# bitsandbytes-foundation/bitsandbytes

Measured on AMD Instinct MI355X. Metric: NF4 gemv_4bit / Linear4bit decode forward GB/s (M=1, N=K=4096; algorithmic bytes / time), higher is better.
Workload: dtype bf16

## Files before the change

### bitsandbytes_amd/cextension.py

```python
from __future__ import annotations

import ctypes as ct
import logging
import os
from pathlib import Path

logger = logging.getLogger(__name__)

PACKAGE_DIR = Path(__file__).resolve().parent
LIB_NAME = "libbitsandbytes_mi355x.so"
LIB_PATH = Path(os.environ.get("BNB_MI355X_LIBRARY", PACKAGE_DIR / LIB_NAME))


class MissingNativeLibrary:

    def __init__(self, reason: str):
        self._reason = reason

    def __getattr__(self, name):
        raise RuntimeError(
            f"bitsandbytes_amd: native symbol '{name}' requested but {LIB_NAME} is not loaded ({self._reason}). "
            f"Build it with `make -C {PACKAGE_DIR / 'csrc'}` (needs hipcc, targets gfx950). "
            "There is no CPU or PyTorch fallback for the 4-bit kernels in this package."
        )
# ... 42 lines not shown
    sig(["bnb_mi355x_gemm_4bit_grad_input_workspace_bytes"], [_I32] * 3, ct.c_size_t)
    sig(["bnb_mi355x_gemm_4bit_grad_input_supported"], [_I32] * 5, _I32)
    sig(["bnb_mi355x_peer_buffer_bytes"], [_I32, ct.c_size_t], ct.c_size_t)
    sig(["bnb_mi355x_peer_alloc"], [ct.c_size_t], _VOID_P)
    sig(["bnb_mi355x_peer_free", "bnb_mi355x_peer_close"], [_VOID_P])
    sig(["bnb_mi355x_peer_export"], [_VOID_P, _VOID_P], _I32)
    sig(["bnb_mi355x_peer_open"], [_VOID_P], _VOID_P)
    sig(["bnb_mi355x_peer_allgather"], [_VOID_P, _I32, _I32, _VOID_P, _VOID_P, ct.c_size_t, ct.c_size_t, _VOID_P])
    sig(["bnb_mi355x_peer_status"], [_VOID_P], _I32)
    sig(["bnb_mi355x_peer_chain_buffer_bytes"], [ct.c_long], ct.c_size_t)
    sig(["bnb_mi355x_peer_chain_alloc"], [ct.c_size_t, _I32], _VOID_P)
    sig(["bnb_mi355x_gemv_4bit_peer_serves"], [_I32] * 5 + [ct.c_long, _I32], _I32)
    sig(["bnb_mi355x_gemv_4bit_peer"], [_VOID_P, _VOID_P, _I32, _I32, _I32] + [_VOID_P] * 8 + [_I32] * 5 + [ct.c_long, _I32, _I32, _VOID_P], _I32)
    sig(["bnb_mi355x_peer_chain_read"], [_VOID_P, _VOID_P, _I32, _I32, _I32, _VOID_P, _I32, ct.c_long, _I32, _VOID_P])
    sig(["bnb_mi355x_set_stream_tuning"], [_I32] * 5)
    sig(["bnb_mi355x_set_tuning"], [_I32] * 4)
    sig(["bnb_mi355x_set_stamp_buffer"], [_VOID_P])
    sig(["bnb_mi355x_version"], [], ct.c_char_p)


def load_native_library():
    if not LIB_PATH.exists():
        return MissingNativeLibrary(f"{LIB_PATH} does not exist")
    try:
        dll = ct.CDLL(str(LIB_PATH))
        _declare(dll)
    except (OSError, AttributeError) as exc:
        logger.error("bitsandbytes_amd: failed to load %s: %s", LIB_PATH, exc)
        return MissingNativeLibrary(str(exc))
    return dll
# ... 5 lines not shown
    [f"cquantize_blockwise_{d}_{q}" for d in ("fp32", "bf16", "fp16") for q in ("nf4", "fp4")]
    + [f"cdequantize_blockwise_{d}_{q}" for d in ("fp32", "bf16", "fp16") for q in ("nf4", "fp4")]
    + [f"cquantize_blockwise_{d}" for d in ("fp32", "bf16", "fp16")]
    + [f"cdequantize_blockwise_{d}" for d in ("fp32", "bf16", "fp16")]
    + [f"cgemm_4bit_{d}" for d in ("fp32", "bf16", "fp16")]
    + [f"cgemm_4bit_inference_naive_{d}" for d in ("fp32", "bf16", "fp16")]
    + ["get_context", "cget_managed_ptr", "bnb_mi355x_quantize_4bit", "bnb_mi355x_quantize_8bit", "bnb_mi355x_quantize_4bit_nested", "bnb_mi355x_dequantize_4bit_nested", "bnb_mi355x_dequantize_4bit_rows",
       "bnb_mi355x_gemm_4bit", "bnb_mi355x_gemm_4bit_workspace_bytes", "bnb_mi355x_gemm_4bit_route", "bnb_mi355x_last_gemm_kernel",
       "bnb_mi355x_gemm_4bit_grouped", "bnb_mi355x_gemm_4bit_grouped_route",
       "bnb_mi355x_gemm_4bit_experts", "bnb_mi355x_gemm_4bit_experts_supported",
       "bnb_mi355x_gemm_4bit_grad_input", "bnb_mi355x_gemm_4bit_grad_input_workspace_bytes", "bnb_mi355x_gemm_4bit_grad_input_supported",
       "bnb_mi355x_peer_buffer_bytes", "bnb_mi355x_peer_alloc", "bnb_mi355x_peer_free", "bnb_mi355x_peer_export", "bnb_mi355x_peer_open",
       "bnb_mi355x_peer_close", "bnb_mi355x_peer_allgather", "bnb_mi355x_peer_status",
       "bnb_mi355x_peer_chain_buffer_bytes", "bnb_mi355x_peer_chain_alloc", "bnb_mi355x_gemv_4bit_peer_serves", "bnb_mi355x_gemv_4bit_peer",
       "bnb_mi355x_peer_chain_read",
       "bnb_mi355x_set_stream_tuning", "bnb_mi355x_set_tuning", "bnb_mi355x_set_stamp_buffer", "bnb_mi355x_version"]
)
```

### bitsandbytes_amd/csrc/c_api.hip

```cpp
#include "bnb_common.h"

#include "../../include/bnb_mi355x.h"

namespace bnb {
void quantize_4bit_f32(const float*, float*, uint8_t*, int, long, int, hipStream_t);
void quantize_4bit_f16(const void*, float*, uint8_t*, int, long, int, hipStream_t);
void quantize_4bit_bf16(const void*, float*, uint8_t*, int, long, int, hipStream_t);
void dequantize_4bit_f32(const uint8_t*, const float*, float*, int, long, int, hipStream_t);
void dequantize_4bit_rows(int, const uint8_t*, const float*, const void*, int, void*, long, long, int, int, int, hipStream_t);
void dequantize_4bit_f16(const uint8_t*, const float*, void*, int, long, int, hipStream_t);
void dequantize_4bit_bf16(const uint8_t*, const float*, void*, int, long, int, hipStream_t);
void quantize_8bit_f32(const float*, const float*, float*, uint8_t*, int, long, hipStream_t);
void quantize_8bit_f16(const float*, const void*, float*, uint8_t*, int, long, hipStream_t);
void quantize_8bit_bf16(const float*, const void*, float*, uint8_t*, int, long, hipStream_t);
void dequantize_8bit_f32(const float*, const uint8_t*, const float*, float*, int, long, hipStream_t);
void dequantize_8bit_f16(const float*, const uint8_t*, const float*, void*, int, long, hipStream_t);
void dequantize_8bit_bf16(const float*, const uint8_t*, const float*, void*, int, long, hipStream_t);
void gemv_4bit_stream(int dtype, const void* A, const uint8_t* B, const float* absmax, const uint8_t* absmax8,
                      const float* absmax_code, const float* absmax_offset, const float* code16, void* out,
                      const void* bias, int M, int N, int K, int blocksize, int quant_type, hipStream_t stream);
bool gemv_4bit_grouped(int dtype, const void* A, int count, const uint8_t* const* B, const float* const* absmax,
                       const uint8_t* const* absmax8, const float* const* absmax_code, const float* const* absmax_offset,
                       void* const* out, const void* const* bias, const int* N, int M, int K, int blocksize, int quant_type,
                       hipStream_t stream);
void gemv_4bit_stream_tuning(int ns, int sw, int rows_per_wg, int nt, int waves);
bool gemv_4bit_peer(void* const* bufs, void* epoch_word, int world, int rank, int dtype, const void* A, const uint8_t* B, const float* absmax,
                    const uint8_t* absmax8, const float* absmax_code, const float* absmax_offset, const void* bias, void* out_local,
                    int ns, int K, int blocksize, int quant_type, int mode, long max_values, int wg_limit, uint32_t epoch_offset,
                    uint32_t spin_bound, hipStream_t stream);
void peer_chain_read(void* const* bufs, void* epoch_word, int world, int rank, int dtype, void* out, int nvalues, long max_values, uint32_t epoch_offset,
                     uint32_t spin_bound, hipStream_t stream);
bool gemv_4bit_peer_serves(int world, int ns, int K, int blocksize, int mode, long max_values, int wg_limit);
thread_local int g_last_gemm_kernel = kKernelNone;
#ifdef BNB_PROFILING
unsigned long long* g_dbg_buf = nullptr;
#endif
bool gemm_4bit_mfma_supported(int dtype, const void* A, const uint8_t* B, const float* code16, int M, int N, int K, int blocksize, bool plain_absmax);
void gemm_4bit_mfma(int dtype, const void* A, const uint8_t* B, const float* absmax, const uint8_t* absmax8,
                    const float* absmax_code, const float* absmax_offset, const float* code16, void* out,
                    const void* bias, int M, int N, int K, int blocksize, int quant_type, void* workspace,
// ... 375 lines not shown
int bnb_mi355x_gemm_4bit_grad_input_supported(int dtype, int M, int N, int K, int blocksize) {
    static const int dummy_aligned[4] __attribute__((aligned(16))) = {0, 0, 0, 0};
    return gemm_4bit_grad_input_supported(dtype, dummy_aligned, reinterpret_cast<const uint8_t*>(dummy_aligned), M, N, K, blocksize) ? 1 : 0;
}
void bnb_mi355x_set_tuning(int reserved0, int reserved1, int mfma_knob0, int mfma_knob1) {
    quantize_8bit_set_variant(reserved0);
    quantize_4bit_set_variant(reserved0 == 3 ? 1 : reserved0 == 4 ? 4 : reserved0 == 5 ? 3 : reserved0 == 8 ? 2 : 0);
    dequantize_4bit_set_variant(reserved0 >= 10 ? reserved0 - 10 : 0);
    gemm_4bit_grad_input_set_slices(reserved1);
    g_mfma_knob0.store(mfma_knob0, std::memory_order_relaxed);
    g_mfma_knob1.store(mfma_knob1, std::memory_order_relaxed);
}
void bnb_mi355x_set_stream_tuning(int ring_depth, int segments, int rows_per_workgroup, int nontemporal, int waves) {
    gemv_4bit_stream_tuning(ring_depth, segments, rows_per_workgroup, nontemporal, waves);
}
void bnb_mi355x_set_stamp_buffer(void* device_u64_buffer) {
#ifdef BNB_PROFILING
    g_dbg_buf = static_cast<unsigned long long*>(device_u64_buffer);
#else
    (void)device_u64_buffer;
#endif
}
const char* bnb_mi355x_version(void) { return "bitsandbytes_amd 0.1.1 gfx950"; }

#pragma GCC visibility pop
}
```

### bitsandbytes_amd/csrc/gemm4_mfma_sm.hip

```cpp
#include "bnb_common.h"

namespace bnb {

#ifdef BNB_PROFILING
extern unsigned long long* g_dbg_buf;
#endif

namespace {

using u32x4 = __attribute__((ext_vector_type(4))) uint32_t;
using f32x4 = __attribute__((ext_vector_type(4))) float;
using i32x4 = __attribute__((ext_vector_type(4))) int;

template <typename T> struct SmMma;
template <> struct SmMma<bf16> {
    using frag = __attribute__((ext_vector_type(8))) bf16;
    static __device__ __forceinline__ f32x4 run(u32x4 a, u32x4 b, f32x4 c) {
        return __builtin_amdgcn_mfma_f32_16x16x32_bf16(__builtin_bit_cast(frag, a), __builtin_bit_cast(frag, b), c, 0, 0, 0);
    }
    static __device__ __forceinline__ uint32_t pack(float first, float second) {
        using V = __attribute__((ext_vector_type(2))) bf16;
        V v;
        v[0] = static_cast<bf16>(first);
        v[1] = static_cast<bf16>(second);
// ... 238 lines not shown
        asm volatile("" : "+s"(ob));
        offset = __builtin_bit_cast(float, ob);
    }

    const int mrow = ln & (SROWS - 1);
    const uint32_t frag_base = stage_lds + static_cast<uint32_t>(mrow * 512) +
                               static_cast<uint32_t>(((4 * (lg & 1) + 2 * (lg >> 1)) ^ sm_swz(mrow)) << 4);
    u32x4 af[8];
    auto read_frags = [&]() {
#pragma unroll
        for (int s = 0; s < 8; ++s) {
            const uint32_t sbits = static_cast<uint32_t>(256 * (s >> 2) + 128 * ((s >> 1) & 1) + 16 * (s & 1));
            af[s] = *reinterpret_cast<const __attribute__((address_space(3))) u32x4*>(frag_base ^ sbits);
        }
    };
    __syncthreads();
    BNB_SM_STAMP(5)
    if constexpr (!SINGLE) {
        issue(st[1], 1);
        __builtin_amdgcn_sched_barrier(0);
    }
    if constexpr (ORDER == 1)
        sm_wait_vm<0>();
    else
        sm_wait_vm<NS * LPS>();
    BNB_SM_STAMP(3)
    read_frags();
    if constexpr (!SINGLE) {
        if (nchunks > 1) {
            sm_wait_lgkm0();
// ... 340 lines not shown
```

### bitsandbytes_amd/csrc/gemv4_stream.hip

```cpp
#include "bnb_common.h"

#include <type_traits>

namespace bnb {

#ifdef BNB_PROFILING
extern unsigned long long* g_dbg_buf;
#endif

namespace {

using u32x4 = __attribute__((ext_vector_type(4))) uint32_t;
using f32x2 = __attribute__((ext_vector_type(2))) float;
using f32x4 = __attribute__((ext_vector_type(4))) float;

typedef __attribute__((address_space(3))) unsigned char* lds_ptr;

constexpr int kSegK = 2048;
constexpr int kLutBytes = 65536;
constexpr int kMaxGroup = 8;

enum StreamFlags : int {
    kNested = 1,
    kCodePtr = 2,
    kFp4 = 4,
    kNT = 8,
    kGrouped = 16,
    kMulti = 32,
    kPeer = 64
};

struct StreamMat {
    const uint8_t* B;
    const float* absmax;
    const uint8_t* absmax8;
    const float* absmax_code;
    const float* absmax_offset;
    void* out;
    const void* bias;
    int N;
    int row_start;
};

#ifdef BNB_PROFILING
// ... 68 lines not shown
    for (int i = 0; i < 4; ++i) {
        const uint32_t e = v[i];
        dst[i] = __builtin_bit_cast(float, e);
    }
}

template <typename T, int MB, int WAVES, int NS, int FLAGS>
__global__ __launch_bounds__(WAVES * 64) __attribute__((amdgpu_waves_per_eu(WAVES / 4, WAVES / 4))) void gemv4_stream_kernel(
    const void* hot_A, const uint8_t* hot_B, const float* hot_absmax, const uint8_t* hot_absmax8, int hot_N, int hot_K,
    int hot_packed , int hot_geom ,
    int hot_inv , const StreamArgs p) {
    constexpr bool NESTED = FLAGS & kNested, CODEPTR = FLAGS & kCodePtr, NT = FLAGS & kNT, GROUPED = FLAGS & kGrouped;
    constexpr bool MULTI = FLAGS & kMulti;
    constexpr bool PEER = (FLAGS & kPeer) != 0;
    static_assert(!PEER || (MB == 1 && !MULTI && !GROUPED && WAVES == 16), "the peer-chain form is the M = 1, single-phase kernel");
    constexpr int THREADS = WAVES * 64;
    constexpr int TB = TypeInfo<T>::bytes;
    constexpr int CH = 2 * TB;
    constexpr int EPC = 16 / TB;
    constexpr int LPS = 2;
    constexpr int BUILDERS = (WAVES >= 16) ? WAVES / 2 : WAVES;
    constexpr int IL = (NS % 2 == 0 && WAVES < 16 && MB <= 2) ? 2 : 1;
    static_assert(NS % IL == 0, "the ring is consumed IL stages at a time");

    extern __shared__ __attribute__((aligned(16))) unsigned char smem[];
    const int tid = threadIdx.x;
    const int lane = tid & 63;
    const int wave = __builtin_amdgcn_readfirstlane(tid >> 6);
    const int K = hot_K;
    const int M = hot_packed & 0x3FFFF, bs_shift = (hot_packed >> 18) & 31, P = MULTI ? (hot_packed >> 23) & 511 : 1;
    const int R = hot_geom & 0xFFFF, SW = (hot_geom >> 16) & 31, G = (hot_geom >> 21) & 31;
    const int S = (K + kSegK - 1) >> 11;
    const int rows_total = GROUPED ? p.rows_total : hot_N;
    const int row_begin = blockIdx.x * R;
    if (row_begin >= rows_total)
        return;
    const int nrows = (rows_total - row_begin < R) ? rows_total - row_begin : R;
    const int m0 = blockIdx.y * MB;
    const int g = (wave * hot_inv) >> 8;
    const int sw = wave - g * SW;
#ifdef BNB_PROFILING
    if (p.dbg && lane == 0)
        BNB_ST_DBG_BASE[(static_cast<long>(blockIdx.x) * WAVES + wave) * 16 + 13] = __builtin_amdgcn_s_memrealtime();
#endif
    BNB_ST_STAMP(0)

    constexpr int kCode2Bytes = (GROUPED ? kMaxGroup : 1) * 1024 + 64;
    float* const code2 = reinterpret_cast<float*>(smem + kLutBytes);
    unsigned char* const ximg = smem + kLutBytes + kCode2Bytes;
    float* const part = reinterpret_cast<float*>(ximg + MB * SW * kSegK * TB);

    const T* __restrict__ A = static_cast<const T*>(hot_A);

    constexpr int C2PASS = (kMaxGroup * 256 + THREADS - 1) / THREADS;
    float code2_v[NESTED ? C2PASS : 1];
// ... 4 lines not shown
#pragma unroll
        for (int i = 0; i < C2PASS; ++i) {
            const int t = i * THREADS + tid;
            code2_v[i] = (t < nmat * 256) ? p.mat[GROUPED ? (t >> 8) : 0].absmax_code[t & 255] : 0.0f;
        }
        offset = p.mat[GROUPED ? (tid < nmat ? tid : 0) : 0].absmax_offset[0];
    }
    float* const offs = reinterpret_cast<float*>(smem + kLutBytes + kCode2Bytes - 64);
    if constexpr (CODEPTR)
        cv = p.code16[lane & 15];

    auto swz = [](int l) -> int { return (CH == 4) ? ((l >> 2) & 3) : ((l >> 1) & 7); };
    auto issue_x = [&](int ph) {
        if (wave >= BUILDERS)
            return;
        const int segs = (S - ph * SW < SW) ? S - ph * SW : SW;
        const int pieces = MB * segs * CH;
        for (int piece = wave; piece < pieces; piece += BUILDERS) {
            const int t = piece / CH, pc = piece - t * CH;
            const int m = (MB == 1) ? 0 : t / segs;
            const int sg = t - m * segs;
            const int s = pc * 64 + lane;
            const int lp = s / CH, j = s - lp * CH;
            const int kl = (CH * lp + (j ^ swz(lp))) * EPC;
            const int k = (ph * SW + sg) * kSegK + kl;
            const int mr = (m0 + m < M) ? m0 + m : M - 1;
            const T* src = A + static_cast<long>(mr) * K + ((k < K) ? k : 0);
            const uint32_t dst = static_cast<uint32_t>(reinterpret_cast<uintptr_t>((lds_ptr)ximg)) +
                                 static_cast<uint32_t>(((m * SW + sg) * CH + pc) * 1024);
            asm volatile("s_mov_b32 m0, %1\n\ts_nop 0\n\tglobal_load_lds_dwordx4 %0, off" : : "v"(src), "s"(dst) : "memory", "m0");
// ... 16 lines not shown
        int mi = 0;
        if constexpr (GROUPED) {
#pragma unroll
            for (int i = 1; i < kMaxGroup; ++i)
                mi = (i < p.nmat && grow >= p.mat[i].row_start) ? i : mi;
        }
        return mi;
    };

    int seg = sw;
    int rl_end = 0;
    uint32_t k0 = 0;
    bool k_ok = false;

    uint32_t lane_mask = kOob;
    auto issue = [&](Stage& s, int i) {
        const bool valid = g + i * G < rl_end;
        const int grow = valid ? row_begin + g + i * G : 0;
        const uint32_t inval = (valid ? 0u : kOob) | lane_mask;
        const uint8_t* Bp = hot_B;
        const float* am = hot_absmax;
        const uint8_t* am8 = hot_absmax8;
        int row = grow;
        if constexpr (GROUPED) {
            const int mi = mat_of(grow);
            Bp = p.mat[mi].B;
            am = p.mat[mi].absmax;
            am8 = p.mat[mi].absmax8;
            row = valid ? grow - p.mat[mi].row_start : 0;
        }
        const auto rs_w = __builtin_amdgcn_make_buffer_rsrc(const_cast<uint8_t*>(Bp), 0, kRecords, kRsrcFlags);
        s.w = __builtin_bit_cast(u32x4, __builtin_amdgcn_raw_buffer_load_b128(
                                            rs_w, (k0 >> 1) | inval,
                                            static_cast<uint32_t>(row) * static_cast<uint32_t>(K >> 1), kWeightAux));
        const uint32_t blk = (static_cast<uint32_t>(row) * static_cast<uint32_t>(K) + k0) >> bs_shift;
        if constexpr (NESTED) {
            const auto rs_q = __builtin_amdgcn_make_buffer_rsrc(const_cast<uint8_t*>(am8), 0, kRecords, kRsrcFlags);
            s.s = __builtin_bit_cast(float, static_cast<uint32_t>(__builtin_amdgcn_raw_buffer_load_b8(rs_q, blk | inval, 0, 0)));
            const uint32_t e0 = static_cast<uint32_t>(row) * static_cast<uint32_t>(K) + static_cast<uint32_t>(seg * kSegK);
            uint32_t k_last = static_cast<uint32_t>(seg * kSegK + kSegK - 1);
            k_last = k_last < static_cast<uint32_t>(K) ? k_last : static_cast<uint32_t>(K - 1);
            const uint32_t e1 = static_cast<uint32_t>(row) * static_cast<uint32_t>(K) + k_last;
            const uint32_t ga = valid && seg < S ? (e0 >> bs_shift) >> 8 : 0u, gb = valid && seg < S ? (e1 >> bs_shift) >> 8 : 0u;
            s.grp = ga;
            typedef const float __attribute__((address_space(4))) * cfloat_ptr;
            const cfloat_ptr amc = (cfloat_ptr)(reinterpret_cast<uintptr_t>(am));
            s.s2a = amc[__builtin_amdgcn_readfirstlane(ga)];
            s.s2b = amc[__builtin_amdgcn_readfirstlane(gb)];
        } else {
            const auto rs_a = __builtin_amdgcn_make_buffer_rsrc(const_cast<float*>(am), 0, kRecords, kRsrcFlags);
            s.s = __builtin_bit_cast(float, __builtin_amdgcn_raw_buffer_load_b32(rs_a, (blk * 4u) | inval, 0, 0));
        }
    };

    uint32_t perm_sel = 0x0C0C0400u;
    const uint32_t lane_off = static_cast<uint32_t>(lane & 31) * 8u;
    f32x2 xr[MB][16];

    auto load_slice = [&]() {
#pragma unroll
        for (int m = 0; m < MB; ++m) {
            float xs[32];
#pragma unroll
            for (int q = 0; q < CH; ++q) {
                const int slot = CH * lane + (q ^ swz(lane));
                const u32x4 v = *reinterpret_cast<const u32x4*>(ximg + ((m * SW + sw) * CH * 64 + slot) * 16);
                unpack16<T>(v, &xs[q * EPC]);
            }
            if ((seg + 1) * kSegK > K) {
#pragma unroll
                for (int e = 0; e < 32; ++e)
                    xs[e] = k_ok ? xs[e] : 0.0f;
            }
#pragma unroll
            for (int b = 0; b < 16; ++b)
                xr[m][b] = f32x2{xs[2 * b], xs[2 * b + 1]};
        }
    };

    auto compute = [&](int j0, int i0) {
        f32x2 pr[IL][16];
        float c2v[IL];
        if constexpr (NESTED) {
#pragma unroll
// ... 25 lines not shown
                int rowl = row_begin + g + (i0 + u) * G;
                int mi = 0;
                if constexpr (GROUPED) {
                    mi = mat_of(rowl);
                    rowl -= p.mat[mi].row_start;
                }
                const uint32_t lane_grp = ((static_cast<uint32_t>(rowl) * static_cast<uint32_t>(K) + k0) >> bs_shift) >> 8;
                const float s2 = lane_grp == s.grp ? s.s2a : s.s2b;
                if constexpr (GROUPED)
                    scale = nested_scale(c2v[u], s2, offs[mi]);
                else
                    scale = nested_scale(c2v[u], s2, offset);
            } else {
                scale = s.s;
            }
            scale_u[u] = k_ok ? scale : 0.0f;
            if constexpr (PRESCALE) {
                const f32x2 sc2 = {scale_u[u], scale_u[u]};
#pragma unroll
                for (int b = 0; b < 16; ++b)
                    pr[u][b] = pr[u][b] * sc2;
            }
        }
        f32x2 acc[IL][MB][2];
#pragma unroll
        for (int u = 0; u < IL; ++u)
#pragma unroll
            for (int m = 0; m < MB; ++m)
                acc[u][m][0] = acc[u][m][1] = f32x2{0.0f, 0.0f};
#pragma unroll
        for (int b = 0; b < 16; ++b)
// ... 3 lines not shown
                for (int m = 0; m < MB; ++m)
                    acc[u][m][b & 1] = __builtin_elementwise_fma(pr[u][b], xr[m][b], acc[u][m][b & 1]);
        float v[IL * MB];
#pragma unroll
        for (int u = 0; u < IL; ++u) {
#pragma unroll
            for (int m = 0; m < MB; ++m) {
                const float sum = (acc[u][m][0][0] + acc[u][m][0][1]) + (acc[u][m][1][0] + acc[u][m][1][1]);
                v[u * MB + m] = PRESCALE ? sum : sum * scale_u[u];
            }
        }
        wave_sum_n<IL * MB>(v);
#pragma unroll
        for (int u = 0; u < IL; ++u) {
            const int rl = g + (i0 + u) * G;
            if (lane == 0 && rl < rl_end) {
#pragma unroll
                for (int m = 0; m < MB; ++m)
                    part[(rl * S + seg) * MB + m] = v[u * MB + m];
            }
        }
    };

    uint32_t epoch = 0;
    uint32_t epoch_raw = 0;
    for (int ph = 0; ph < P; ++ph) {
        if (ph > 0)
            __syncthreads();
        if (ph == 0)
            BNB_ST_STAMP(9)
        bool x_from_peer = false;
        u32x4 gx[PEER ? kChainRounds : 1];
        if constexpr (PEER) {
            const int peer_mode = (hot_packed >> 24) & 15;
            x_from_peer = (peer_mode & 1) != 0;
            if (x_from_peer && wave < WAVES - BUILDERS) {
                const auto rs_x = __builtin_amdgcn_make_buffer_rsrc(const_cast<void*>(hot_A), 0, K * 4, kRsrcFlags);
#pragma unroll
                for (int r = 0; r < kChainRounds; ++r)
                    gx[r] = __builtin_bit_cast(u32x4, __builtin_amdgcn_raw_buffer_load_b128(
                                                          rs_x, static_cast<uint32_t>((r * (WAVES - BUILDERS) + wave) * 64 + lane) * 16u, 0, 17 ));
            }
        }
        if (!x_from_peer)
            issue_x(ph);
        if (ph == 0)
            BNB_ST_STAMP(10)
        seg = ph * SW + sw;
        rl_end = (g < G && seg < S) ? nrows : 0;
        k0 = static_cast<uint32_t>(seg * kSegK + lane * 32);
        k_ok = (seg < S) && (k0 < static_cast<uint32_t>(K));
        lane_mask = k_ok ? 0u : kOob;
#pragma unroll
        for (int j = 0; j < NS; ++j) {
            issue(st[j], j);
            __builtin_amdgcn_sched_barrier(0);
        }
        if constexpr (PEER) {
            typedef const uint32_t __attribute__((address_space(4))) * cu32_ptr;
            epoch_raw = *(cu32_ptr)(reinterpret_cast<uintptr_t>(p.peer.epoch_word));
            epoch = epoch_raw + p.peer.epoch_offset;
        }
        if (ph == 0)
            BNB_ST_STAMP(1)
        if (ph == 0) {
            __builtin_amdgcn_sched_barrier(0);
        }
        const bool table_builder = (PEER && x_from_peer) ? (wave >= WAVES - BUILDERS) : (wave < BUILDERS);
        const int tid_b = (PEER && x_from_peer) ? tid - (WAVES - BUILDERS) * 64 : tid;
        if (ph == 0 && table_builder) {
            if constexpr (!CODEPTR)
                cv = code_literal<(FLAGS & kFp4) != 0>((lane & 15) + opaque_zero());
            constexpr int BT = BUILDERS * 64;
            constexpr int ITERS = kLutBytes / 16 / BT;
            static_assert((kLutBytes / 16) % BT == 0 && BT % 256 == 0, "whole passes over the table");
            const int cvb = __builtin_bit_cast(int, cv);
            const float lo = __builtin_bit_cast(float, __builtin_amdgcn_ds_bpermute(((tid_b >> 4) & 15) * 4, cvb));
            float hi[ITERS];
#pragma unroll
            for (int it = 0; it < ITERS; ++it)
                hi[it] = __builtin_bit_cast(float, __builtin_amdgcn_ds_bpermute(((it * BT + tid_b) >> 8) * 4, cvb));
// ... 50 lines not shown
                auto put4 = [&](uint32_t j4, u32x2 four) {
                    const uint32_t c = j4 >> 1, half = j4 & 1u;
                    const uint32_t sg = c >> 8, cs = c & 255u, lp = cs / CH, q = cs % CH;
                    *reinterpret_cast<u32x2*>(ximg + ((sg * CH * 64 + CH * lp + (q ^ static_cast<uint32_t>(swz(static_cast<int>(lp))))) * 16 + half * 8)) = four;
                };
#pragma unroll
                for (int r = 0; r < kChainRounds; ++r) {
                    const uint32_t off = static_cast<uint32_t>((r * (WAVES - BUILDERS) + wave) * 64 + lane) * 16u;
                    if (off < static_cast<uint32_t>(K) * 4u) {
                        const u32x4 gr = settle(gx[r], off);
                        put4(off >> 4, u32x2{gr[0], gr[2]});
                    }
                }
            }
        }
        __syncthreads();
        if (ph == 0)
            BNB_ST_STAMP(3)
        perm_sel = 0x0C0C0400u + static_cast<uint32_t>(opaque_zero());
        load_slice();
        if (ph == 0)
            BNB_ST_STAMP(4)
#ifdef BNB_PROFILING
        if (ph == 0 && p.dbg && !(reinterpret_cast<uintptr_t>(p.dbg) & 1)) {
            asm volatile("s_waitcnt vmcnt(%0)" ::"n"(NS * LPS - 1) : "memory");
            BNB_ST_STAMP(15)
        }
#endif
        int base = 0;
        for (; g + (base + NS) * G < rl_end; base += NS) {
#pragma unroll
            for (int j = 0; j < NS; j += IL) {
                compute(j, base + j);
                if (ph == 0 && base == 0 && j == 0)
                    BNB_ST_STAMP(5)
#pragma unroll
                for (int u = 0; u < IL; ++u)
                    issue(st[j + u], base + j + u + NS);
            }
        }
#pragma unroll
        for (int j = 0; j < NS; j += IL) {
            if (g + (base + j) * G < rl_end)
                compute(j, base + j);
            if (ph == 0 && base == 0 && j == 0)
                BNB_ST_STAMP(5)
        }
    }
    BNB_ST_STAMP(6)
    if (reinterpret_cast<uintptr_t>((lds_ptr)smem) != 0)
        __builtin_trap();

    [[maybe_unused]] uint32_t epoch_out = 0;
    if constexpr (PEER)
        epoch_out = epoch + 1u;
    __syncthreads();
    BNB_ST_STAMP(7)
    for (int idx = tid; idx < nrows * MB; idx += THREADS) {
        const int m = (MB == 1) ? 0 : idx / nrows, rl = idx - m * nrows;
        if (m0 + m >= M)
            continue;
        float v = 0.0f;
        for (int sg = 0; sg < S; ++sg)
            v += part[(rl * S + sg) * MB + m];
        const int grow = row_begin + rl;
        int mi = 0, row = grow;
        if constexpr (GROUPED) {
            mi = mat_of(grow);
            row = grow - p.mat[mi].row_start;
        }
        const T* bias = static_cast<const T*>(p.mat[mi].bias);
        const float b = bias ? static_cast<float>(bias[row]) : 0.0f;
        const T tv = static_cast<T>(v + b);
        if constexpr (PEER) {
            if (p.mat[mi].out != nullptr)
                static_cast<T*>(p.mat[mi].out)[row] = tv;
            if (p.peer.mode & 2) {
                const uint32_t own = static_cast<uint32_t>(__builtin_bit_cast(unsigned short, tv));
                const uint32_t other = static_cast<uint32_t>(__builtin_amdgcn_ds_bpermute((lane ^ 1) << 2, static_cast<int>(own)));
                const uint32_t pair = own | (other << 16);
                const uint32_t pair2 = static_cast<uint32_t>(__builtin_amdgcn_ds_bpermute((lane ^ 2) << 2, static_cast<int>(pair)));
                const size_t slot = kChainDataOffset + (static_cast<size_t>((p.peer.epoch_offset + 1u) & (kChainRegions - 1u)) * p.peer.max_granules +
                                                        ((static_cast<size_t>(p.peer.rank) * static_cast<size_t>(rows_total) + static_cast<size_t>(row)) >> 1)) * 8u;
                if (p.peer.mode & 8) {
                    const float gf = static_cast<float>(tv), uf = static_cast<float>(__builtin_bit_cast(T, static_cast<unsigned short>(other)));
                    const T st = static_cast<T>(gf / (1.0f + expf(-gf)));
                    const T at = static_cast<T>(__fmul_rn(static_cast<float>(st), uf));
                    const uint32_t abits = static_cast<uint32_t>(__builtin_bit_cast(unsigned short, at));
                    const uint32_t anext = static_cast<uint32_t>(__builtin_amdgcn_ds_bpermute((lane ^ 2) << 2, static_cast<int>(abits)));
                    if (!(row & 3)) {
                        using u32x2 = __attribute__((ext_vector_type(2))) uint32_t;
// ... 20 lines not shown
                        }
                    }
                } else if (!(row & 1)) {
                    using u32x2 = __attribute__((ext_vector_type(2))) uint32_t;
                    const u32x2 granule = {pair, epoch_out};
                    for (int pr = 0; pr < p.peer.world; ++pr) {
                        unsigned char* const dst = p.peer.base[pr] + slot;
                        if (pr == p.peer.rank)
                            asm volatile("global_store_dwordx2 %0, %1, off" ::"v"(dst), "v"(granule) : "memory");
                        else
                            asm volatile("global_store_dwordx2 %0, %1, off sc0 sc1" ::"v"(dst), "v"(granule) : "memory");
                    }
                }
            }
        } else {
            static_cast<T*>(p.mat[mi].out)[static_cast<long>(m0 + m) * p.mat[mi].N + row] = tv;
        }
    }
    BNB_ST_STAMP(8)
#ifdef BNB_PROFILING
    if (p.dbg && lane == 0)
        BNB_ST_DBG_BASE[(static_cast<long>(blockIdx.x) * WAVES + wave) * 16 + 14] = __builtin_amdgcn_s_memrealtime();
#endif
}

struct GenericArgs {
    const void* A;
    const uint8_t* B;
    const float* absmax;
    const uint8_t* absmax8;
    const float* absmax_code;
// ... 88 lines not shown
    ge.R = R;
    ge.P = (S + sw - 1) / sw;
    ge.grid_x = (rows_total + R - 1) / R;
    ge.lds = fixed + ((static_cast<size_t>(R) * S * mb * 4 + 15) & ~size_t(15)) + ximg;
    return ge;
}

struct StreamTuning {
    TlsKnob ns{0}, sw{0}, rows{0}, nt{-1}, waves{0};
};
thread_local StreamTuning g_tune;

constexpr int kRing = 2;
constexpr int ring_depth(int mb, int waves) { return (mb == 1 && waves == 8) ? 4 : kRing; }

template <typename T, int MB, int WAVES, int NS, int FLAGS> void launch_one(const StreamArgs& a, hipStream_t stream) {
    const Geometry ge = make_geometry(a.rows_total, a.K, MB, WAVES, TypeInfo<T>::bytes, (FLAGS & kGrouped) != 0, g_tune.sw.load(std::memory_order_relaxed),
                                      g_tune.rows.load(std::memory_order_relaxed));
    dim3 grid(ge.grid_x, (a.M + MB - 1) / MB);
    const StreamMat& m0 = a.mat[0];
    if constexpr (!(FLAGS & kGrouped) && NS == ring_depth(MB, WAVES) && !(MB == 2 && WAVES == 16)) {
        if (ge.P > 1) {
            auto kern = gemv4_stream_kernel<T, MB, WAVES, NS, FLAGS | kMulti>;
            static LdsLimit lds_limit;
            ensure_dynamic_lds(lds_limit, reinterpret_cast<const void*>(kern), ge.lds);
            hipLaunchKernelGGL(kern, grid, dim3(WAVES * 64), ge.lds, stream, a.A, m0.B, m0.absmax, m0.absmax8, m0.N, a.K,
                               (a.M & 0x3FFFF) | (a.bs_shift << 18) | (ge.P << 23),
                               ge.R | (ge.SW << 16) | (ge.G << 21), (256 + ge.SW - 1) / ge.SW, a);
            return;
        }
    }
    if (ge.P > 1) {
        if constexpr (!(FLAGS & kGrouped) && (NS != ring_depth(MB, WAVES) || (MB == 2 && WAVES == 16)))
            return launch_one<T, MB, (MB == 1 ? 16 : 8), kRing, FLAGS | kNT>(a, stream);
        fprintf(stderr, "bitsandbytes_amd: gemv_4bit: internal error, multi-phase geometry on a single-phase instance\n");
        exit(1);
    }
    auto kern = gemv4_stream_kernel<T, MB, WAVES, NS, FLAGS>;
    static LdsLimit lds_limit;
    ensure_dynamic_lds(lds_limit, reinterpret_cast<const void*>(kern), ge.lds);
    hipLaunchKernelGGL(kern, grid, dim3(WAVES * 64), ge.lds, stream, a.A, m0.B, m0.absmax, m0.absmax8, m0.N, a.K,
                       (a.M & 0x3FFFF) | (a.bs_shift << 18) | (ge.P << 23),
                       ge.R | (ge.SW << 16) | (ge.G << 21), (256 + ge.SW - 1) / ge.SW, a);
}

template <typename T, int MB, int WAVES, int FLAGS> void launch_tuned(const StreamArgs& a, hipStream_t stream) {
    if constexpr (std::is_same<T, bf16>::value && MB == 1 && FLAGS == 0) {
        const int ns = g_tune.ns.load(std::memory_order_relaxed);
        const int nt = g_tune.nt.load(std::memory_order_relaxed);
        if constexpr (WAVES == 8) {
            if (ns == 2)
                return launch_one<T, 1, 8, 2, kNT>(a, stream);
            if (nt == 0)
                return launch_one<T, 1, 8, 4, 0>(a, stream);
        } else {
            if (ns == 4)
                return launch_one<T, 1, 16, 4, kNT>(a, stream);
            if (ns == 3)
// ... 224 lines not shown
    pc.world = world;
    pc.rank = rank;
    pc.max_granules = static_cast<uint32_t>(max_values / 2);
    pc.spin_bound = spin_bound;
    pc.epoch_offset = epoch_offset;
    pc.mode = 0;
    const int granules = (nvalues + 1) / 2;
    const int grid = (granules + 255) / 256 < 8 ? (granules + 255) / 256 : 8;
    if (dtype == 2)
        hipLaunchKernelGGL(peer_chain_read_kernel<bf16>, dim3(grid > 0 ? grid : 1), dim3(256), 0, stream, pc, static_cast<bf16*>(out), nvalues);
    else
        hipLaunchKernelGGL(peer_chain_read_kernel<f16>, dim3(grid > 0 ? grid : 1), dim3(256), 0, stream, pc, static_cast<f16*>(out), nvalues);
    BNB_CHECK_LAUNCH();
}

void gemv_4bit_stream_tuning(int ns, int sw, int rows_per_wg, int nt, int waves) {
    g_tune.ns.store(ns, std::memory_order_relaxed);
    g_tune.sw.store(sw, std::memory_order_relaxed);
    g_tune.rows.store(rows_per_wg, std::memory_order_relaxed);
    g_tune.nt.store(nt, std::memory_order_relaxed);
    g_tune.waves.store(waves, std::memory_order_relaxed);
}

void gemv_4bit_stream(int dtype, const void* A, const uint8_t* B, const float* absmax, const uint8_t* absmax8,
                   const float* absmax_code, const float* absmax_offset, const float* code16, void* out,
                   const void* bias, int M, int N, int K, int blocksize, int quant_type, hipStream_t stream) {
    if (M <= 0 || N <= 0 || K <= 0)
        return;
    if (stream_ok(A, M, K, blocksize) && aligned_to(B, 16)) {
        StreamArgs a;
// ... 72 lines not shown
```

### include/bnb_mi355x.h

```cpp
#ifndef BNB_MI355X_H
#define BNB_MI355X_H

#include <stddef.h>
#include <stdint.h>

#ifdef __cplusplus
extern "C" {
#endif

typedef void* bnb_stream_t;

void cquantize_blockwise_fp32_nf4(float* code, float* A, float* absmax, unsigned char* out, int blocksize, const int n);
void cquantize_blockwise_fp32_fp4(float* code, float* A, float* absmax, unsigned char* out, int blocksize, const int n);
void cquantize_blockwise_fp16_nf4(float* code, void* A, float* absmax, unsigned char* out, int blocksize, const int n);
void cquantize_blockwise_fp16_fp4(float* code, void* A, float* absmax, unsigned char* out, int blocksize, const int n);
void cquantize_blockwise_bf16_nf4(float* code, void* A, float* absmax, unsigned char* out, int blocksize, const int n);
void cquantize_blockwise_bf16_fp4(float* code, void* A, float* absmax, unsigned char* out, int blocksize, const int n);

void cdequantize_blockwise_fp32_nf4(float* code, unsigned char* A, float* absmax, float* out, int blocksize, const int n, bnb_stream_t stream);
void cdequantize_blockwise_fp32_fp4(float* code, unsigned char* A, float* absmax, float* out, int blocksize, const int n, bnb_stream_t stream);
void cdequantize_blockwise_fp16_nf4(float* code, unsigned char* A, float* absmax, void* out, int blocksize, const int n, bnb_stream_t stream);
void cdequantize_blockwise_fp16_fp4(float* code, unsigned char* A, float* absmax, void* out, int blocksize, const int n, bnb_stream_t stream);
void cdequantize_blockwise_bf16_nf4(float* code, unsigned char* A, float* absmax, void* out, int blocksize, const int n, bnb_stream_t stream);
void cdequantize_blockwise_bf16_fp4(float* code, unsigned char* A, float* absmax, void* out, int blocksize, const int n, bnb_stream_t stream);
// ... 48 lines not shown
void* bnb_mi355x_peer_open(const void* handle64);
void bnb_mi355x_peer_close(void* mapped);
void bnb_mi355x_peer_allgather(void* const* bufs, int world, int rank, const void* src, void* out, size_t bytes, size_t max_bytes, bnb_stream_t stream);
int bnb_mi355x_peer_status(const void* local_buffer);

size_t bnb_mi355x_peer_chain_buffer_bytes(long max_values);
void* bnb_mi355x_peer_chain_alloc(size_t bytes, int fine_grained);
int bnb_mi355x_gemv_4bit_peer_serves(int world, int ns, int K, int blocksize, int mode, long max_values, int wg_limit);
int bnb_mi355x_gemv_4bit_peer(void* const* bufs, void* epoch_word, int world, int rank, int dtype, const void* A, const uint8_t* B, const float* absmax, const uint8_t* absmax_8bit, const float* absmax_code, const float* absmax_offset, const void* bias, void* out_local, int ns, int K, int blocksize, int quant_type, int mode, long max_values, int wg_limit, int epoch_offset, bnb_stream_t stream);
void bnb_mi355x_peer_chain_read(void* const* bufs, void* epoch_word, int world, int rank, int dtype, void* out, int nvalues, long max_values, int epoch_offset, bnb_stream_t stream);

void bnb_mi355x_set_tuning(int reserved0, int reserved1, int mfma_knob0, int mfma_knob1);

void bnb_mi355x_set_stream_tuning(int ring_depth, int segments, int rows_per_workgroup, int nontemporal, int waves);

void bnb_mi355x_set_stamp_buffer(void* device_u64_buffer);

const char* bnb_mi355x_version(void);

#ifdef __cplusplus
}
#endif

#endif
```

Measured before the change: 2316.

## Add exact-geometry M=1 gemv stream kernel variant and early epilogue pointer loads

Adds a compile-time 'exact' instantiation of the 4-bit stream GEMV for M=1 with 16-bit activations and K of exactly two 2048-wide segments. It hard-codes K, segment count and wave grouping, drops the row and K bounds checks and masking, and loads the activation vector straight into LDS with global_load_lds. It also reads the output and bias pointers early and pins them in scalar registers, so the epilogue does not reload kernel arguments. A tuning knob can select a late-args twin or the general path instead, and a new C API query reports whether the exact path applies. The cost is extra kernel instantiations and a narrow path that runs only when the geometry divides evenly.

```diff
diff --git a/bitsandbytes_amd/cextension.py b/bitsandbytes_amd/cextension.py
--- a/bitsandbytes_amd/cextension.py
+++ b/bitsandbytes_amd/cextension.py
@@ -80,6 +80,7 @@
     sig(["bnb_mi355x_gemv_4bit_peer"], [_VOID_P, _VOID_P, _I32, _I32, _I32] + [_VOID_P] * 8 + [_I32] * 5 + [ct.c_long, _I32, _I32, _VOID_P], _I32)
     sig(["bnb_mi355x_peer_chain_read"], [_VOID_P, _VOID_P, _I32, _I32, _I32, _VOID_P, _I32, ct.c_long, _I32, _VOID_P])
     sig(["bnb_mi355x_set_stream_tuning"], [_I32] * 5)
+    sig(["bnb_mi355x_gemv_4bit_stream_exact"], [_I32] * 6, _I32)
     sig(["bnb_mi355x_set_tuning"], [_I32] * 4)
     sig(["bnb_mi355x_set_stamp_buffer"], [_VOID_P])
     sig(["bnb_mi355x_version"], [], ct.c_char_p)
@@ -115,5 +116,5 @@
        "bnb_mi355x_peer_close", "bnb_mi355x_peer_allgather", "bnb_mi355x_peer_status",
        "bnb_mi355x_peer_chain_buffer_bytes", "bnb_mi355x_peer_chain_alloc", "bnb_mi355x_gemv_4bit_peer_serves", "bnb_mi355x_gemv_4bit_peer",
        "bnb_mi355x_peer_chain_read",
-       "bnb_mi355x_set_stream_tuning", "bnb_mi355x_set_tuning", "bnb_mi355x_set_stamp_buffer", "bnb_mi355x_version"]
+       "bnb_mi355x_set_stream_tuning", "bnb_mi355x_gemv_4bit_stream_exact", "bnb_mi355x_set_tuning", "bnb_mi355x_set_stamp_buffer", "bnb_mi355x_version"]
 )
diff --git a/bitsandbytes_amd/csrc/c_api.hip b/bitsandbytes_amd/csrc/c_api.hip
--- a/bitsandbytes_amd/csrc/c_api.hip
+++ b/bitsandbytes_amd/csrc/c_api.hip
@@ -24,6 +24,7 @@
                        void* const* out, const void* const* bias, const int* N, int M, int K, int blocksize, int quant_type,
                        hipStream_t stream);
 void gemv_4bit_stream_tuning(int ns, int sw, int rows_per_wg, int nt, int waves);
+bool gemv_4bit_stream_exact(int dtype, int M, int N, int K, int blocksize, bool nested);
 bool gemv_4bit_peer(void* const* bufs, void* epoch_word, int world, int rank, int dtype, const void* A, const uint8_t* B, const float* absmax,
                     const uint8_t* absmax8, const float* absmax_code, const float* absmax_offset, const void* bias, void* out_local,
                     int ns, int K, int blocksize, int quant_type, int mode, long max_values, int wg_limit, uint32_t epoch_offset,
@@ -429,6 +430,9 @@
 void bnb_mi355x_set_stream_tuning(int ring_depth, int segments, int rows_per_workgroup, int nontemporal, int waves) {
     gemv_4bit_stream_tuning(ring_depth, segments, rows_per_workgroup, nontemporal, waves);
 }
+int bnb_mi355x_gemv_4bit_stream_exact(int dtype, int M, int N, int K, int blocksize, int nested) {
+    return gemv_4bit_stream_exact(dtype, M, N, K, blocksize, nested != 0) ? 1 : 0;
+}
 void bnb_mi355x_set_stamp_buffer(void* device_u64_buffer) {
 #ifdef BNB_PROFILING
     g_dbg_buf = static_cast<unsigned long long*>(device_u64_buffer);
diff --git a/bitsandbytes_amd/csrc/gemm4_mfma_sm.hip b/bitsandbytes_amd/csrc/gemm4_mfma_sm.hip
--- a/bitsandbytes_amd/csrc/gemm4_mfma_sm.hip
+++ b/bitsandbytes_amd/csrc/gemm4_mfma_sm.hip
@@ -276,6 +276,8 @@
             af[s] = *reinterpret_cast<const __attribute__((address_space(3))) u32x4*>(frag_base ^ sbits);
         }
     };
+    if constexpr (!GROUPED)
+        asm volatile("" : "+s"(g_out), "+s"(g_bias));
     __syncthreads();
     BNB_SM_STAMP(5)
     if constexpr (!SINGLE) {
diff --git a/bitsandbytes_amd/csrc/gemv4_stream.hip b/bitsandbytes_amd/csrc/gemv4_stream.hip
--- a/bitsandbytes_amd/csrc/gemv4_stream.hip
+++ b/bitsandbytes_amd/csrc/gemv4_stream.hip
@@ -27,7 +27,9 @@
     kNT = 8,
     kGrouped = 16,
     kMulti = 32,
-    kPeer = 64
+    kPeer = 64,
+    kExact = 128,
+    kLateArgs = 256
 };
 
 struct StreamMat {
@@ -126,6 +128,11 @@
     constexpr bool MULTI = FLAGS & kMulti;
     constexpr bool PEER = (FLAGS & kPeer) != 0;
     static_assert(!PEER || (MB == 1 && !MULTI && !GROUPED && WAVES == 16), "the peer-chain form is the M = 1, single-phase kernel");
+    constexpr bool EXACT = (FLAGS & kExact) != 0;
+    constexpr int kExactSW = 2;
+    static_assert(!EXACT || (MB == 1 && !MULTI && !GROUPED && !PEER && !CODEPTR && WAVES == 16 && TypeInfo<T>::bytes == 2),
+                  "the exact-geometry form is the M = 1, single-phase kernel for 16-bit activations");
+    constexpr bool EARLY_ARGS = !GROUPED && !(FLAGS & kLateArgs);
     constexpr int THREADS = WAVES * 64;
     constexpr int TB = TypeInfo<T>::bytes;
     constexpr int CH = 2 * TB;
@@ -139,18 +146,20 @@
     const int tid = threadIdx.x;
     const int lane = tid & 63;
     const int wave = __builtin_amdgcn_readfirstlane(tid >> 6);
-    const int K = hot_K;
-    const int M = hot_packed & 0x3FFFF, bs_shift = (hot_packed >> 18) & 31, P = MULTI ? (hot_packed >> 23) & 511 : 1;
-    const int R = hot_geom & 0xFFFF, SW = (hot_geom >> 16) & 31, G = (hot_geom >> 21) & 31;
-    const int S = (K + kSegK - 1) >> 11;
+    const int K = EXACT ? kExactSW * kSegK : hot_K;
+    const int M = EXACT ? 1 : hot_packed & 0x3FFFF, bs_shift = (hot_packed >> 18) & 31, P = MULTI ? (hot_packed >> 23) & 511 : 1;
+    const int R = hot_geom & 0xFFFF, SW = EXACT ? kExactSW : (hot_geom >> 16) & 31, G = EXACT ? WAVES / kExactSW : (hot_geom >> 21) & 31;
+    const int S = EXACT ? kExactSW : (K + kSegK - 1) >> 11;
     const int rows_total = GROUPED ? p.rows_total : hot_N;
     const int row_begin = blockIdx.x * R;
-    if (row_begin >= rows_total)
-        return;
-    const int nrows = (rows_total - row_begin < R) ? rows_total - row_begin : R;
-    const int m0 = blockIdx.y * MB;
-    const int g = (wave * hot_inv) >> 8;
-    const int sw = wave - g * SW;
+    if constexpr (!EXACT) {
+        if (row_begin >= rows_total)
+            return;
+    }
+    const int nrows = (EXACT || rows_total - row_begin >= R) ? R : rows_total - row_begin;
+    const int m0 = EXACT ? 0 : blockIdx.y * MB;
+    const int g = EXACT ? wave / kExactSW : (wave * hot_inv) >> 8;
+    const int sw = EXACT ? wave % kExactSW : wave - g * SW;
 #ifdef BNB_PROFILING
     if (p.dbg && lane == 0)
         BNB_ST_DBG_BASE[(static_cast<long>(blockIdx.x) * WAVES + wave) * 16 + 13] = __builtin_amdgcn_s_memrealtime();
@@ -185,6 +194,14 @@
     auto issue_x = [&](int ph) {
         if (wave >= BUILDERS)
             return;
+        if constexpr (EXACT) {
+            static_assert(kExactSW * CH == BUILDERS && CH == 4, "one piece per builder wavefront");
+            const unsigned char* const src = reinterpret_cast<const unsigned char*>(A) + wave * 1024;
+            const uint32_t voff = static_cast<uint32_t>(lane ^ ((lane >> 4) & 3)) * 16u;
+            const uint32_t dst = static_cast<uint32_t>(reinterpret_cast<uintptr_t>((lds_ptr)ximg)) + static_cast<uint32_t>(wave * 1024);
+            asm volatile("s_mov_b32 m0, %2\n\ts_nop 0\n\tglobal_load_lds_dwordx4 %0, %1" : : "v"(voff), "s"(src), "s"(dst) : "memory", "m0");
+            return;
+        }
         const int segs = (S - ph * SW < SW) ? S - ph * SW : SW;
         const int pieces = MB * segs * CH;
         for (int piece = wave; piece < pieces; piece += BUILDERS) {
@@ -231,8 +248,8 @@
     bool k_ok = false;
 
     uint32_t lane_mask = kOob;
-    auto issue = [&](Stage& s, int i) {
-        const bool valid = g + i * G < rl_end;
+    auto issue = [&](Stage& s, int i, auto first) {
+        const bool valid = (EXACT && decltype(first)::value) || g + i * G < rl_end;
         const int grow = valid ? row_begin + g + i * G : 0;
         const uint32_t inval = (valid ? 0u : kOob) | lane_mask;
         const uint8_t* Bp = hot_B;
@@ -258,7 +275,7 @@
             uint32_t k_last = static_cast<uint32_t>(seg * kSegK + kSegK - 1);
             k_last = k_last < static_cast<uint32_t>(K) ? k_last : static_cast<uint32_t>(K - 1);
             const uint32_t e1 = static_cast<uint32_t>(row) * static_cast<uint32_t>(K) + k_last;
-            const uint32_t ga = valid && seg < S ? (e0 >> bs_shift) >> 8 : 0u, gb = valid && seg < S ? (e1 >> bs_shift) >> 8 : 0u;
+            const uint32_t ga = valid && (EXACT || seg < S) ? (e0 >> bs_shift) >> 8 : 0u, gb = valid && (EXACT || seg < S) ? (e1 >> bs_shift) >> 8 : 0u;
             s.grp = ga;
             typedef const float __attribute__((address_space(4))) * cfloat_ptr;
             const cfloat_ptr amc = (cfloat_ptr)(reinterpret_cast<uintptr_t>(am));
@@ -284,7 +301,7 @@
                 const u32x4 v = *reinterpret_cast<const u32x4*>(ximg + ((m * SW + sw) * CH * 64 + slot) * 16);
                 unpack16<T>(v, &xs[q * EPC]);
             }
-            if ((seg + 1) * kSegK > K) {
+            if (!EXACT && (seg + 1) * kSegK > K) {
 #pragma unroll
                 for (int e = 0; e < 32; ++e)
                     xs[e] = k_ok ? xs[e] : 0.0f;
@@ -340,7 +357,7 @@
             } else {
                 scale = s.s;
             }
-            scale_u[u] = k_ok ? scale : 0.0f;
+            scale_u[u] = (EXACT || k_ok) ? scale : 0.0f;
             if constexpr (PRESCALE) {
                 const f32x2 sc2 = {scale_u[u], scale_u[u]};
 #pragma unroll
@@ -374,7 +391,7 @@
 #pragma unroll
         for (int u = 0; u < IL; ++u) {
             const int rl = g + (i0 + u) * G;
-            if (lane == 0 && rl < rl_end) {
+            if (lane == 0 && (EXACT || rl < rl_end)) {
 #pragma unroll
                 for (int m = 0; m < MB; ++m)
                     part[(rl * S + seg) * MB + m] = v[u * MB + m];
@@ -382,6 +399,7 @@
         }
     };
 
+    [[maybe_unused]] uintptr_t ep_out = 0, ep_bias = 0;
     uint32_t epoch = 0;
     uint32_t epoch_raw = 0;
     for (int ph = 0; ph < P; ++ph) {
@@ -407,13 +425,13 @@
         if (ph == 0)
             BNB_ST_STAMP(10)
         seg = ph * SW + sw;
-        rl_end = (g < G && seg < S) ? nrows : 0;
+        rl_end = (EXACT || (g < G && seg < S)) ? nrows : 0;
         k0 = static_cast<uint32_t>(seg * kSegK + lane * 32);
-        k_ok = (seg < S) && (k0 < static_cast<uint32_t>(K));
+        k_ok = EXACT || ((seg < S) && (k0 < static_cast<uint32_t>(K)));
         lane_mask = k_ok ? 0u : kOob;
 #pragma unroll
         for (int j = 0; j < NS; ++j) {
-            issue(st[j], j);
+            issue(st[j], j, std::true_type{});
             __builtin_amdgcn_sched_barrier(0);
         }
         if constexpr (PEER) {
@@ -425,6 +443,11 @@
             BNB_ST_STAMP(1)
         if (ph == 0) {
             __builtin_amdgcn_sched_barrier(0);
+            if constexpr (EARLY_ARGS) {
+                ep_out = reinterpret_cast<uintptr_t>(p.mat[0].out);
+                ep_bias = reinterpret_cast<uintptr_t>(p.mat[0].bias);
+                __builtin_amdgcn_sched_barrier(0);
+            }
         }
         const bool table_builder = (PEER && x_from_peer) ? (wave >= WAVES - BUILDERS) : (wave < BUILDERS);
         const int tid_b = (PEER && x_from_peer) ? tid - (WAVES - BUILDERS) * 64 : tid;
@@ -505,6 +528,10 @@
                 }
             }
         }
+        if constexpr (EARLY_ARGS) {
+            if (ph == 0)
+                asm volatile("" : "+s"(ep_out), "+s"(ep_bias));
+        }
         __syncthreads();
         if (ph == 0)
             BNB_ST_STAMP(3)
@@ -519,7 +546,7 @@
         }
 #endif
         int base = 0;
-        for (; g + (base + NS) * G < rl_end; base += NS) {
+        for (; EXACT ? (base + NS) * G < R : g + (base + NS) * G < rl_end; base += NS) {
 #pragma unroll
             for (int j = 0; j < NS; j += IL) {
                 compute(j, base + j);
@@ -527,12 +554,12 @@
                     BNB_ST_STAMP(5)
 #pragma unroll
                 for (int u = 0; u < IL; ++u)
-                    issue(st[j + u], base + j + u + NS);
+                    issue(st[j + u], base + j + u + NS, std::false_type{});
             }
         }
 #pragma unroll
         for (int j = 0; j < NS; j += IL) {
-            if (g + (base + j) * G < rl_end)
+            if (EXACT ? (base + j) * G < R : g + (base + j) * G < rl_end)
                 compute(j, base + j);
             if (ph == 0 && base == 0 && j == 0)
                 BNB_ST_STAMP(5)
@@ -560,12 +587,14 @@
             mi = mat_of(grow);
             row = grow - p.mat[mi].row_start;
         }
-        const T* bias = static_cast<const T*>(p.mat[mi].bias);
+        const T* bias = EARLY_ARGS ? reinterpret_cast<const T*>(ep_bias) : static_cast<const T*>(p.mat[mi].bias);
+        T* const out = EARLY_ARGS ? reinterpret_cast<T*>(ep_out) : static_cast<T*>(p.mat[mi].out);
+        const int out_n = GROUPED ? p.mat[mi].N : hot_N;
         const float b = bias ? static_cast<float>(bias[row]) : 0.0f;
         const T tv = static_cast<T>(v + b);
         if constexpr (PEER) {
-            if (p.mat[mi].out != nullptr)
-                static_cast<T*>(p.mat[mi].out)[row] = tv;
+            if (out != nullptr)
+                out[row] = tv;
             if (p.peer.mode & 2) {
                 const uint32_t own = static_cast<uint32_t>(__builtin_bit_cast(unsigned short, tv));
                 const uint32_t other = static_cast<uint32_t>(__builtin_amdgcn_ds_bpermute((lane ^ 1) << 2, static_cast<int>(own)));
@@ -616,7 +645,7 @@
                 }
             }
         } else {
-            static_cast<T*>(p.mat[mi].out)[static_cast<long>(m0 + m) * p.mat[mi].N + row] = tv;
+            out[static_cast<long>(m0 + m) * out_n + row] = tv;
         }
     }
     BNB_ST_STAMP(8)
@@ -735,21 +764,43 @@
 constexpr int kRing = 2;
 constexpr int ring_depth(int mb, int waves) { return (mb == 1 && waves == 8) ? 4 : kRing; }
 
+constexpr int kExactSegments = 2;
+bool exact_geometry(const Geometry& ge, int M, int rows_total, int K, int ns) {
+    return M == 1 && ge.P == 1 && K == kExactSegments * kSegK && ge.SW == kExactSegments && ge.G == 16 / kExactSegments &&
+           rows_total % ge.R == 0 && ge.R % ge.G == 0 && ge.R >= ns * ge.G;
+}
+template <typename T, int MB, int WAVES, int NS, int FLAGS> constexpr bool has_exact_twin() {
+    return TypeInfo<T>::bytes == 2 && MB == 1 && WAVES == 16 && NS == kRing && (FLAGS & ~kFp4) == kNT;
+}
+constexpr int kTuneGeneral = 2, kTuneLateArgs = 3;
+
 template <typename T, int MB, int WAVES, int NS, int FLAGS> void launch_one(const StreamArgs& a, hipStream_t stream) {
     const Geometry ge = make_geometry(a.rows_total, a.K, MB, WAVES, TypeInfo<T>::bytes, (FLAGS & kGrouped) != 0, g_tune.sw.load(std::memory_order_relaxed),
                                       g_tune.rows.load(std::memory_order_relaxed));
     dim3 grid(ge.grid_x, (a.M + MB - 1) / MB);
     const StreamMat& m0 = a.mat[0];
+    auto go = [&](auto kern) {
+        static LdsLimit lds_limit;
+        ensure_dynamic_lds(lds_limit, reinterpret_cast<const void*>(kern), ge.lds);
+        hipLaunchKernelGGL(kern, grid, dim3(WAVES * 64), ge.lds, stream, a.A, m0.B, m0.absmax, m0.absmax8, m0.N, a.K,
+                           (a.M & 0x3FFFF) | (a.bs_shift << 18) | (ge.P << 23),
+                           ge.R | (ge.SW << 16) | (ge.G << 21), (256 + ge.SW - 1) / ge.SW, a);
+    };
+    constexpr bool kLateTwin = std::is_same<T, bf16>::value && MB == 1 && WAVES == 16 && NS == kRing && (FLAGS == kNT || FLAGS == (kNT | kFp4 | kNested));
+    if constexpr (has_exact_twin<T, MB, WAVES, NS, FLAGS>() || kLateTwin) {
+        const int knob = g_tune.nt.load(std::memory_order_relaxed);
+        if constexpr (kLateTwin) {
+            if (knob == kTuneLateArgs && ge.P == 1)
+                return go(gemv4_stream_kernel<T, MB, WAVES, NS, FLAGS | kLateArgs>);
+        }
+        if constexpr (has_exact_twin<T, MB, WAVES, NS, FLAGS>()) {
+            if (knob != kTuneGeneral && knob != kTuneLateArgs && exact_geometry(ge, a.M, a.rows_total, a.K, NS))
+                return go(gemv4_stream_kernel<T, MB, WAVES, NS, FLAGS | kExact>);
+        }
+    }
     if constexpr (!(FLAGS & kGrouped) && NS == ring_depth(MB, WAVES) && !(MB == 2 && WAVES == 16)) {
-        if (ge.P > 1) {
-            auto kern = gemv4_stream_kernel<T, MB, WAVES, NS, FLAGS | kMulti>;
-            static LdsLimit lds_limit;
-            ensure_dynamic_lds(lds_limit, reinterpret_cast<const void*>(kern), ge.lds);
-            hipLaunchKernelGGL(kern, grid, dim3(WAVES * 64), ge.lds, stream, a.A, m0.B, m0.absmax, m0.absmax8, m0.N, a.K,
-                               (a.M & 0x3FFFF) | (a.bs_shift << 18) | (ge.P << 23),
-                               ge.R | (ge.SW << 16) | (ge.G << 21), (256 + ge.SW - 1) / ge.SW, a);
-            return;
-        }
+        if (ge.P > 1)
+            return go(gemv4_stream_kernel<T, MB, WAVES, NS, FLAGS | kMulti>);
     }
     if (ge.P > 1) {
         if constexpr (!(FLAGS & kGrouped) && (NS != ring_depth(MB, WAVES) || (MB == 2 && WAVES == 16)))
@@ -757,12 +808,7 @@
         fprintf(stderr, "bitsandbytes_amd: gemv_4bit: internal error, multi-phase geometry on a single-phase instance\n");
         exit(1);
     }
-    auto kern = gemv4_stream_kernel<T, MB, WAVES, NS, FLAGS>;
-    static LdsLimit lds_limit;
-    ensure_dynamic_lds(lds_limit, reinterpret_cast<const void*>(kern), ge.lds);
-    hipLaunchKernelGGL(kern, grid, dim3(WAVES * 64), ge.lds, stream, a.A, m0.B, m0.absmax, m0.absmax8, m0.N, a.K,
-                       (a.M & 0x3FFFF) | (a.bs_shift << 18) | (ge.P << 23),
-                       ge.R | (ge.SW << 16) | (ge.G << 21), (256 + ge.SW - 1) / ge.SW, a);
+    go(gemv4_stream_kernel<T, MB, WAVES, NS, FLAGS>);
 }
 
 template <typename T, int MB, int WAVES, int FLAGS> void launch_tuned(const StreamArgs& a, hipStream_t stream) {
@@ -1017,6 +1063,16 @@
     BNB_CHECK_LAUNCH();
 }
 
+bool gemv_4bit_stream_exact(int dtype, int M, int N, int K, int blocksize, bool nested) {
+    const int knob = g_tune.nt.load(std::memory_order_relaxed);
+    if (nested || (dtype != 1 && dtype != 2) || M != 1 || N <= 0 || K <= 0 || K % 32 != 0 || blocksize < 32 || !is_pow2(blocksize) ||
+        g_tune.waves.load(std::memory_order_relaxed) == 8 || g_tune.ns.load(std::memory_order_relaxed) != 0 || knob == 0 || knob == kTuneGeneral ||
+        knob == kTuneLateArgs)
+        return false;
+    const Geometry ge = make_geometry(N, K, 1, 16, 2, false, g_tune.sw.load(std::memory_order_relaxed), g_tune.rows.load(std::memory_order_relaxed));
+    return exact_geometry(ge, M, N, K, kRing);
+}
+
 void gemv_4bit_stream_tuning(int ns, int sw, int rows_per_wg, int nt, int waves) {
     g_tune.ns.store(ns, std::memory_order_relaxed);
     g_tune.sw.store(sw, std::memory_order_relaxed);
diff --git a/include/bnb_mi355x.h b/include/bnb_mi355x.h
--- a/include/bnb_mi355x.h
+++ b/include/bnb_mi355x.h
@@ -86,6 +86,8 @@
 
 void bnb_mi355x_set_stream_tuning(int ring_depth, int segments, int rows_per_workgroup, int nontemporal, int waves);
 
+int bnb_mi355x_gemv_4bit_stream_exact(int dtype, int M, int N, int K, int blocksize, int nested);
+
 void bnb_mi355x_set_stamp_buffer(void* device_u64_buffer);
 
 const char* bnb_mi355x_version(void);
```

After: 2564, median of 6. 1.11x the previous value.
